# go-compression/raisin

Measured on AMD Instinct MI355X. Metric: encode+decode MB/s, higher is better.
Workload: dtype u8; 1 GPU; huffman encode+decode, 1024 MiB uniform-random bytes 0x00-0x7F (BASELINE configs[1]), splitmix64 seed 0x5EED0002; algorithm=huffman, bytes_per_gpu=1073741824, chunks=1

## Files before the change

### raisin_amd/csrc/huff_decode.hip

```cpp
#include <chrono>
#include <optional>
#include "codecs.h"
#include "rsn_helpers.h"

namespace rsn {


constexpr int DB = 256;
constexpr int FDB = 256;
constexpr int SW = 8;
constexpr int SBITS = SW * 32;
constexpr int ORG_WORDS = 8;
constexpr int ORG = ORG_WORDS * 32;
constexpr int DATA_WORDS = ORG_WORDS + DB * SW + 8;
constexpr int LUT_BITS_MAX = 11;
constexpr int LUT_WORDS = 1 << LUT_BITS_MAX;
constexpr int OUT_STAGE = DB * 64;
constexpr int OUT_STAGE_RUNE = 40960;
constexpr int CHILD_LDS = 256;
constexpr int LUT2_LDS = 768;
constexpr uint32_t LUT2_GLOBAL_MAX = 1u << 20;
constexpr int SYNC_ROUNDS = 24;
constexpr uint32_t BAD_REL = 0xFFFF;
constexpr uint32_t BAD_POS = 0xFFFFFFFFu;
// ... 582 lines not shown
        for (uint32_t k = 0; k < cnt; k++) dst[k] = (uint8_t)(o[k >> 2] >> (8 * (k & 3)));
    }
    }
    __syncthreads();
    }
}

namespace {

void build_tables(const HuffTree &t, int K, std::vector<uint32_t> &lut, std::vector<int32_t> &child) {
    const uint32_t A = t.n_leaves;
    const size_t n_int = t.freq.size() - A;
    child.assign(2 * std::max<size_t>(n_int, 1), 0);
    for (size_t i = 0; i < n_int; i++) {
        const int32_t id = (int32_t)(A + i);
        const int32_t kids[2] = {t.left[id], t.right[id]};
        for (int b = 0; b < 2; b++)
            child[2 * i + b] = t.is_leaf(kids[b]) ? -(int32_t)(t.rune[kids[b]] + 1) : kids[b] - (int32_t)A;
    }
    lut.assign((size_t)1 << K, 0);
    struct It { int32_t node; uint32_t prefix; int depth; };
    std::vector<It> st;
    st.push_back({t.root, 0, 0});
    while (!st.empty()) {
        const It it = st.back();
        st.pop_back();
        if (t.is_leaf(it.node)) {
            const uint32_t ent = ((uint32_t)it.depth << 24) | t.rune[it.node];
            const uint32_t lo = it.prefix << (K - it.depth);
            for (uint32_t x = 0; x < (1u << (K - it.depth)); x++) lut[lo + x] = ent;
        } else if (it.depth == K) {
            lut[it.prefix] = 0x80000000u | (uint32_t)(it.node - (int32_t)A);
        } else {
            st.push_back({t.right[it.node], (it.prefix << 1) | 1, it.depth + 1});
            st.push_back({t.left[it.node], it.prefix << 1, it.depth + 1});
        }
    }
}

void build_second_level(const std::vector<int32_t> &child, int K, bool byte_alphabet, std::vector<uint32_t> &lut, std::vector<uint32_t> &lut2) {
    lut2.clear();
    const size_t n_int = child.size() / 2;
    std::vector<uint8_t> depth(n_int, 0);
    for (size_t i = 0; i < n_int; i++) {
        unsigned d = 0;
        for (int b = 0; b < 2; b++) { const int32_t k = child[2 * i + b]; d = std::max(d, k < 0 ? 1u : 1u + depth[(size_t)k]); }
        depth[i] = (uint8_t)std::min(d, 255u);
    }
    std::vector<uint32_t> longs;
    for (uint32_t v = 0; v < (1u << K); v++) if (lut[v] & 0x80000000u) longs.push_back(v);
    if (longs.empty()) return;
    auto total = [&](unsigned cap) { uint64_t t = 0; for (uint32_t v : longs) t += 1ull << std::min<unsigned>(depth[lut[v] & 0x3FFFFFFu], cap); return t; };
    unsigned cap = 32u - (unsigned)K;
    if (total(cap) > (uint64_t)LUT2_LDS) {
        const uint64_t budget = byte_alphabet ? (uint64_t)LUT2_LDS : (uint64_t)LUT2_GLOBAL_MAX;
        while (cap > 0 && total(cap) > budget) cap--;
    }
    if (cap == 0) return;
    struct It { int32_t node; uint32_t path; unsigned q; };
    std::vector<It> st;
    for (uint32_t v : longs) {
        const int32_t top = (int32_t)(lut[v] & 0x3FFFFFFu);
        const unsigned sb = std::min<unsigned>(depth[(size_t)top], cap);
        const uint32_t off = (uint32_t)lut2.size();
        lut2.resize(lut2.size() + ((size_t)1 << sb));
        st.push_back({top, 0, 0});
        while (!st.empty()) {
            const It it = st.back();
            st.pop_back();
            if (it.q == sb) { lut2[off + it.path] = 0x80000000u | (uint32_t)it.node; continue; }
            for (int b = 0; b < 2; b++) {
                const int32_t k = child[2 * (size_t)it.node + b];
                const uint32_t path = it.path | ((uint32_t)b << it.q);
                const unsigned q1 = it.q + 1;
                if (k >= 0) { st.push_back({k, path, q1}); continue; }
                const uint32_t ent = ((uint32_t)(K + q1) << 24) | (uint32_t)(-(k + 1));
                for (uint32_t y = 0; y < (1u << (sb - q1)); y++) lut2[off + path + (y << q1)] = ent;
            }
        }
        lut[v] = 0x80000000u | (sb << 26) | off;
    }
}

int rep_for(int K) {
    int r = 0;
    while (r < 5 && ((1 << K) << (r + 1)) <= LUT_WORDS) r++;
    return r;
}

}

int huff_decode_dev(Ctx &c, hipStream_t s, const uint8_t *d_in, size_t n, uint8_t *d_out, size_t out_cap, size_t *out_n, const SliceStream *st) {
    if (((uintptr_t)d_in & 15) || ((uintptr_t)d_out & 15)) return c.fail(RSN_ERR_ARG, "huffman: device buffers must be 16-byte aligned");
    *out_n = 0;
    std::vector<uint8_t> head;
    size_t sep = (size_t)-1;
    for (size_t want = 4096;; want *= 8) {
        const size_t k = std::min(want, n);
        const size_t old = head.size();
        if (k > old) {
            if (st && !st->need_in(k)) return c.fail(RSN_ERR_DEVICE, "huffman: the upload of a sliced call failed");
            void *hpin; int prc = pinned_buf(c, k - old + 64, &hpin); if (prc) return prc;
            RSN_HIP(copy_async(hpin, d_in + old, k - old, hipMemcpyDeviceToHost, s));
            RSN_HIP(hipStreamSynchronize(s));
            head.resize(k);
            memcpy(head.data() + old, hpin, k - old);
        }
        for (size_t i = old ? old - 1 : 0; i + 1 < k; i++) if (head[i] == 0x5C && head[i + 1] == 0x0A) { sep = i; break; }
        if (sep != (size_t)-1 || k == n) break;
    }
    if (sep == (size_t)-1) return c.fail(RSN_ERR_FORMAT, "huffman: no '\\\\\\n' separator (reference: index out of range, huffman.go:264)");
    if (sep + 3 > head.size() && sep + 3 <= n) {
        const size_t old = head.size();
        if (st && !st->need_in(sep + 3)) return c.fail(RSN_ERR_DEVICE, "huffman: the upload of a sliced call failed");
        void *hpin; int prc = pinned_buf(c, 64, &hpin); if (prc) return prc;
        RSN_HIP(copy_async(hpin, d_in + old, sep + 3 - old, hipMemcpyDeviceToHost, s));
        RSN_HIP(hipStreamSynchronize(s));
        head.resize(sep + 3);
        memcpy(head.data() + old, hpin, sep + 3 - old);
    }
    std::vector<HuffSym> syms; std::string msg;
    static const bool host_timing = getenv("RSN_HOST_TIMING") != nullptr;
    auto now = [] { return std::chrono::steady_clock::now(); };
    auto ms = [](std::chrono::steady_clock::time_point a, std::chrono::steady_clock::time_point b) { return std::chrono::duration<double, std::milli>(b - a).count(); };
    const auto t0 = now();
    if (!parse_header(head.data(), sep, syms, msg)) return c.fail(RSN_ERR_FORMAT, "%s", msg.c_str());
    const auto t1 = now();
    const size_t sn = n - sep - 2;
    const unsigned diff = sn ? head[sep + 2] : 0;
    const unsigned long long nbits = sn ? (unsigned long long)(sn - 1) * 8 : 0;
    if (diff > nbits) return c.fail(RSN_ERR_FORMAT, "huffman: pad exceeds the payload (reference: slice bounds out of range, huffman.go:294)");
    const unsigned long long max = nbits - diff;
    if (!d_out) {
        if (syms.empty()) return c.fail(RSN_ERR_FORMAT, "huffman: empty header (reference panics in heap.Pop, huffman.go:102)");
        if (syms.size() == 1) {
            if (max > 0) return c.fail(RSN_ERR_FORMAT, "huffman: single-symbol tree with a non-empty payload (reference recurses without end, huffman.go:139-140)");
            *out_n = 32;
            return c.fail(RSN_ERR_CAPACITY, "huffman: output needs %d bytes by the header's counts", utf8_len(syms[0].rune));
        }
        if (max == 0) return c.fail(RSN_ERR_FORMAT, "huffman: payload ends inside a codeword (reference: index out of range, huffman.go:145)");
        unsigned long long total = 0, expect = 0;
        bool beyond = false;
        for (const HuffSym &sy : syms) {
            if (sy.freq > max - total) { beyond = true; break; }
            total += sy.freq;
            expect += sy.freq * (unsigned long long)utf8_len(sy.rune);
        }
        if (beyond) expect = 4 * max;
        *out_n = round_up((size_t)expect, 16) + 16;
        return c.fail(RSN_ERR_CAPACITY, beyond ? "huffman: output needs at most %llu bytes (the header counts more symbols than the payload holds)"
                                               : "huffman: output needs %llu bytes by the header's counts", expect);
    }
    HuffTree tree; HuffCodes codes;
    if (!build_tree(syms, tree, msg)) return c.fail(RSN_ERR_FORMAT, "%s", msg.c_str());
    const auto t2 = now();
    constexpr int k_env = LUT_BITS_MAX;
    std::vector<uint32_t> lut, lut2; std::vector<int32_t> child;
    const bool prebuilt = tree.n_leaves > 4096;
    std::optional<SideJob> table_builder;
    if (prebuilt) table_builder.emplace([&] { build_tables(tree, k_env, lut, child); build_second_level(child, k_env, false, lut, lut2); });
    const bool codes_ok = assign_codes(tree, codes, msg, false);
    if (prebuilt) table_builder->finish();
    if (!codes_ok) return c.fail(RSN_ERR_LIMIT, "%s", msg.c_str());
    const auto t3 = now();
    if (host_timing) fprintf(stderr, "huffman decode host: header of %zu bytes parsed in %.2f ms, tree %.2f ms, codes %.2f ms, %zu symbols\n", sep, ms(t0, t1), ms(t1, t2), ms(t2, t3), syms.size());

    if (tree.n_leaves == 1) {
        if (max > 0) return c.fail(RSN_ERR_FORMAT, "huffman: single-symbol tree with a non-empty payload (reference recurses without end, huffman.go:139-140)");
        uint8_t u[4];
        const size_t k = (size_t)go_encode_rune(tree.rune[0], u);
        *out_n = k;
        if (!d_out || out_cap < k) { return c.fail(RSN_ERR_CAPACITY, "huffman: output needs %zu bytes", k); }
        RSN_HIP(copy_async(d_out, u, k, hipMemcpyHostToDevice, s));
        RSN_HIP(hipStreamSynchronize(s));
        return RSN_OK;
    }
    if (max == 0) return c.fail(RSN_ERR_FORMAT, "huffman: payload ends inside a codeword (reference: index out of range, huffman.go:145)");

    bool ascii = true;
    for (uint32_t i = 0; i < tree.n_leaves; i++) if (tree.rune[i] >= 0x80) ascii = false;
    const size_t pay = sep + 3;
    const size_t A0 = pay & ~(size_t)15;
    void *p; int rc;

    static const bool no_flat = getenv("RSN_NO_FLAT") != nullptr;
    if (ascii && codes.min_len == codes.max_len && codes.max_len <= 7 && !no_flat) {
        const uint32_t L = codes.max_len;
        if (max % L) return c.fail(RSN_ERR_FORMAT, "huffman: payload ends inside a codeword (reference: index out of range, huffman.go:145)");
        const unsigned long long n_sym = max / L;
// ... 284 lines not shown
```

### raisin_amd/csrc/huff_encode.hip

```cpp
#include <chrono>
#include <cstddef>

#include <optional>
#include "codecs.h"
#include "rsn_helpers.h"

namespace rsn {

constexpr int TILE = 65536;
constexpr int SMALL_TILE = 4096;
constexpr size_t SMALL_INPUT = (size_t)2 << 20;
constexpr size_t RUNE_SMALL_INPUT = (size_t)16 << 20;
constexpr int HB = 256;
constexpr int ROUND = HB * 16;

enum { MODE_ASCII = 0, MODE_ASCII_WIDE = 1, MODE_RUNE = 2 };

template <int INFLIGHT, int TB>
__global__ __launch_bounds__(HB) void k_byte_hist(const uint8_t *__restrict__ in, size_t n, uint32_t n_tiles,
                                                  uint32_t *__restrict__ tile_hist,
                                                  unsigned long long *__restrict__ ghist) {
    __shared__ uint32_t h[128 * 32];
    const int tid = threadIdx.x;
    const uint32_t copy = tid & 31;
    unsigned long long mine = 0;
    uint32_t hi_any = 0;
    static_assert(TB % ROUND == 0 && (TB / ROUND) % INFLIGHT == 0, "whole rounds, whole batches of loads");
    auto add16 = [&](const uint4 &v) {
        const uint32_t w[4] = {v.x, v.y, v.z, v.w};
#pragma unroll
        for (int j = 0; j < 4; j++) {
            hi_any |= w[j];
            atomicAdd(&h[((w[j] & 0x7F) << 5) | copy], 1u);
            atomicAdd(&h[(((w[j] >> 8) & 0x7F) << 5) | copy], 1u);
            atomicAdd(&h[(((w[j] >> 16) & 0x7F) << 5) | copy], 1u);
            atomicAdd(&h[(((w[j] >> 24) & 0x7F) << 5) | copy], 1u);
        }
    };
    for (uint32_t t = blockIdx.x; t < n_tiles; t += gridDim.x) {
        for (int i = tid; i < 128 * 32; i += HB) h[i] = 0;
        __syncthreads();
        const size_t base = (size_t)t * TB;
        if (base + TB <= n) {
            const uint4 *src = reinterpret_cast<const uint4 *>(in + base) + tid;
#pragma unroll
            for (int k0 = 0; k0 < TB / ROUND; k0 += INFLIGHT) {
                uint4 v[INFLIGHT];
#pragma unroll
                for (int k = 0; k < INFLIGHT; k++) v[k] = ld16<(RSN_NT_MASK & 1) != 0>(src + (k0 + k) * HB);
#pragma unroll
                for (int k = 0; k < INFLIGHT; k++) add16(v[k]);
            }
        } else {
            for (int k = 0; k < TB / ROUND; k++) {
                const size_t off = base + (size_t)(k * HB + tid) * 16;
                if (off + 16 <= n) add16(*reinterpret_cast<const uint4 *>(in + off));
                else if (off < n) for (size_t p = off; p < n; p++) { hi_any |= in[p]; atomicAdd(&h[((in[p] & 0x7F) << 5) | copy], 1u); }
            }
        }
        __syncthreads();
        if (tid < 128) {
            uint32_t s = 0;
#pragma unroll
            for (int r = 0; r < 32; r++) s += h[(tid << 5) | ((r + tid) & 31)];
            tile_hist[(size_t)t * 128 + tid] = s;
            mine += s;
        }
        __syncthreads();
    }
    if (tid < 128 && mine) atomicAdd(&ghist[tid], mine);
    if (hi_any & 0x80808080u) atomicAdd(&ghist[128], 1ull);
}

template <int COPIES, int INFLIGHT>
__global__ __launch_bounds__(HB) void k_byte_hist256(const uint8_t *__restrict__ in, size_t n, uint32_t n_tiles,
                                                     unsigned long long *__restrict__ ghist) {
    static_assert(HB == 256 && (COPIES == 16 || COPIES == 32) && (TILE / ROUND) % INFLIGHT == 0, "a thread per bin, whole batches of loads");
    constexpr uint32_t FOLD = 1024;
    constexpr int LOG = COPIES == 32 ? 5 : 4;
    __shared__ uint32_t h[256 * COPIES];
    const int tid = threadIdx.x;
    const uint32_t copy = tid & (COPIES - 1);
    unsigned long long mine = 0;
    auto add16 = [&](const uint4 &v) {
        const uint32_t w[4] = {v.x, v.y, v.z, v.w};
#pragma unroll
        for (int j = 0; j < 4; j++) {
            atomicAdd(&h[((w[j] & 0xFF) << LOG) | copy], 1u);
            atomicAdd(&h[(((w[j] >> 8) & 0xFF) << LOG) | copy], 1u);
            atomicAdd(&h[(((w[j] >> 16) & 0xFF) << LOG) | copy], 1u);
            atomicAdd(&h[((w[j] >> 24) << LOG) | copy], 1u);
        }
    };
    auto fold = [&] {
        __syncthreads();
        uint32_t s = 0;
#pragma unroll
        for (int r = 0; r < COPIES; r++) s += h[(tid << LOG) | ((r + tid) & (COPIES - 1))];
        mine += s;
        __syncthreads();
        for (int i = tid; i < 256 * COPIES; i += HB) h[i] = 0;
        __syncthreads();
    };
    for (int i = tid; i < 256 * COPIES; i += HB) h[i] = 0;
    __syncthreads();
    uint32_t since = 0;
    for (uint32_t t = blockIdx.x; t < n_tiles; t += gridDim.x) {
        const size_t base = (size_t)t * TILE;
        if (base + TILE <= n) {
            const uint4 *src = reinterpret_cast<const uint4 *>(in + base) + tid;
#pragma unroll
            for (int k0 = 0; k0 < TILE / ROUND; k0 += INFLIGHT) {
                uint4 v[INFLIGHT];
#pragma unroll
                for (int k = 0; k < INFLIGHT; k++) v[k] = ld16<true>(src + (k0 + k) * HB);
#pragma unroll
                for (int k = 0; k < INFLIGHT; k++) add16(v[k]);
            }
        } else {
            for (int k = 0; k < TILE / ROUND; k++) {
                const size_t off = base + (size_t)(k * HB + tid) * 16;
                if (off + 16 <= n) add16(*reinterpret_cast<const uint4 *>(in + off));
                else if (off < n) for (size_t p = off; p < n; p++) atomicAdd(&h[((uint32_t)in[p] << LOG) | copy], 1u);
            }
        }
        if (++since == FOLD) { fold(); since = 0; }
    }
    fold();
    if (mine) atomicAdd(&ghist[tid], mine);
}

template <int INFLIGHT>
__global__ __launch_bounds__(HB) void k_bytes_differ(const uint8_t *__restrict__ a, const uint8_t *__restrict__ b, size_t n, uint32_t n_tiles,
                                                     unsigned long long *__restrict__ first) {
    static_assert((TILE / ROUND) % INFLIGHT == 0, "whole batches of loads");
    constexpr unsigned long long NONE = ~0ull;
    __shared__ unsigned long long s_pub, s_min;
    const int tid = threadIdx.x;
    auto diff16 = [](const uint4 &x, const uint4 &y) -> uint32_t {
        const uint32_t d[4] = {x.x ^ y.x, x.y ^ y.y, x.z ^ y.z, x.w ^ y.w};
        uint32_t at = 16;
#pragma unroll
        for (int j = 3; j >= 0; j--) if (d[j]) at = 4 * j + ((uint32_t)__ffs((int)d[j]) - 1) / 8;
        return at;
    };
    for (uint32_t t = blockIdx.x; t < n_tiles; t += gridDim.x) {
        const size_t base = (size_t)t * TILE;
        if (tid == 0) { s_pub = __hip_atomic_load(first, __ATOMIC_RELAXED, __HIP_MEMORY_SCOPE_AGENT); s_min = NONE; }
        __syncthreads();
        if (base >= s_pub) return;
        unsigned long long mine = NONE;
        if (base + TILE <= n) {
            const uint4 *pa = reinterpret_cast<const uint4 *>(a + base) + tid, *pb = reinterpret_cast<const uint4 *>(b + base) + tid;
#pragma unroll
// ... 624 lines not shown
            const int bp = k * L, wi = bp >> 5, sh = bp & 31;
            if (sh + L <= 32) v[wi] |= code << (32 - sh - L);
            else { v[wi] |= code >> (sh + L - 32); v[wi + 1 < L ? wi + 1 : wi] |= code << (64 - sh - L); }
        }
    };
    uint32_t v[L];
    if (s0 < a.n) pack32(s0, v);
    else {
#pragma unroll
        for (int j = 0; j < L; j++) v[j] = 0;
    }
    uint32_t prev = (uint32_t)__builtin_amdgcn_update_dpp(0, (int)v[L - 1], 0x138, 0xF, 0xF, false);
    if (lane == 63) s_last[wv] = v[L - 1];
    __syncthreads();
    if (lane == 0) {
        if (wv > 0) prev = s_last[wv - 1];
        else if (chunk > 0) { uint32_t pv[L]; pack32(s0 - 32, pv); prev = pv[L - 1]; }
        else prev = 0;
    }
    const uint32_t o0 = (uint32_t)(a.base_bits & 31);
#pragma unroll
    for (int j = 0; j < L; j++) {
        const uint32_t hi = j ? v[j - 1] : prev;
        const uint32_t ow = (uint32_t)((((unsigned long long)hi << 32) | v[j]) >> o0);
        const uint32_t i = tid * L + j;
        s_o[i + (i >> 5)] = __builtin_bswap32(ow);
    }
    __syncthreads();
    const unsigned long long total_syms = a.n;
    const unsigned long long wbase = (a.base_bits >> 5) + (unsigned long long)chunk * (HB * L);
    const unsigned long long end_word = (a.base_bits + total_syms * L + 31) >> 5;
    if (chunk > 0 && wbase + (unsigned long long)(HB * L) <= end_word) {
        for (int q = tid; q < HB * L / 4; q += HB) {
            const int i = 4 * q;
            const uint32_t *sp = s_o + i + (i >> 5);
            st16_a4<(RSN_NT_MASK & 4) != 0>(a.out_words + wbase + i, sp[0], sp[1], sp[2], sp[3]);
        }
    } else
    for (int i = tid; i < HB * L; i += HB) {
        const unsigned long long g = wbase + i;
        if (g >= end_word) break;
        const uint32_t val = s_o[i + (i >> 5)];
        if (g == (a.base_bits >> 5)) {
            uint32_t hb = 0;
            for (uint32_t k = (uint32_t)(g * 4); k < a.hdr_len; k++) hb |= (uint32_t)tab[128 + k] << (8 * (k & 3));
            a.out_words[g] = val | hb;
        } else a.out_words[g] = val;
    }
    if (o0 && tid == HB - 1) {
        const unsigned long long g = wbase + (unsigned long long)(HB * L);
        const bool last_block = chunk + 1 == n_chunks;
        if (last_block && g < end_word) a.out_words[g] = __builtin_bswap32(v[L - 1] << (32 - o0));
    }
    __syncthreads();
    }
    if (blockIdx.x == 0) {
        const uint32_t whole = (uint32_t)(a.base_bits >> 5) * 4;
        uint8_t *o8 = reinterpret_cast<uint8_t *>(a.out_words);
        for (uint32_t k = tid; k < whole && k < a.hdr_len; k += HB) o8[k] = tab[128 + k];
    }
}

namespace {

__global__ void k_rune_flags(const unsigned long long *__restrict__ hist, unsigned long long *__restrict__ flag) {
    const uint32_t r = blockIdx.x * blockDim.x + threadIdx.x;
    if (r < kMaxRune) flag[r] = hist[r] != 0;
}
__global__ void k_rune_pairs(const unsigned long long *__restrict__ hist, const unsigned long long *__restrict__ off, HuffSym *__restrict__ out) {
    const uint32_t r = blockIdx.x * blockDim.x + threadIdx.x;
    if (r < kMaxRune && hist[r]) { out[off[r]].rune = r; out[off[r]].freq = hist[r]; }
}
struct RuneCode { uint32_t rune, len; unsigned long long code; };
__global__ void k_rune_table(const RuneCode *__restrict__ list, uint32_t k, unsigned long long *__restrict__ code64, uint8_t *__restrict__ len8) {
    const uint32_t i = blockIdx.x * blockDim.x + threadIdx.x;
    if (i < k) { const RuneCode e = list[i]; code64[e.rune] = e.code; len8[e.rune] = (uint8_t)e.len; }
}

int hist_ascii_or_rune(Ctx &c, hipStream_t s, const uint8_t *d_in, size_t n, uint32_t n_tiles, uint32_t tile, uint32_t *d_tile_hist,
                       std::vector<HuffSym> &syms, bool &ascii, uint16_t **smask_out) {
    void *p;
    int rc = dev_buf(c, 1, 256 * 8, &p); if (rc) return rc;
    unsigned long long *d_gh = (unsigned long long *)p;
    RSN_HIP(hipMemsetAsync(d_gh, 0, 256 * 8, s));
    dim3 grid;
    if (tile == TILE) {
        rc = persistent_grid(c, reinterpret_cast<const void *>(k_byte_hist<4, TILE>), HB, n_tiles, &grid); if (rc) return rc;
        RSN_LAUNCH("huff_byte_hist", (k_byte_hist<4, TILE>), grid, dim3(HB), 0, s, d_in, n, n_tiles, d_tile_hist, d_gh);
    } else {
        rc = persistent_grid(c, reinterpret_cast<const void *>(k_byte_hist<1, SMALL_TILE>), HB, n_tiles, &grid); if (rc) return rc;
        RSN_LAUNCH("huff_byte_hist", (k_byte_hist<1, SMALL_TILE>), grid, dim3(HB), 0, s, d_in, n, n_tiles, d_tile_hist, d_gh);
    }
    void *hp; rc = pinned_buf(c, 256 * 8, &hp); if (rc) return rc;
    unsigned long long *h = (unsigned long long *)hp;
    RSN_HIP(copy_async(h, d_gh, 256 * 8, hipMemcpyDeviceToHost, s));
    RSN_HIP(hipStreamSynchronize(s));
    ascii = h[128] == 0;
    syms.clear();
    if (ascii) {
        for (uint32_t b = 0; b < 128; b++) if (h[b]) syms.push_back({b, h[b]});
        return RSN_OK;
    }
    rc = dev_buf(c, 2, (size_t)kMaxRune * 8, &p); if (rc) return rc;
    unsigned long long *d_rh = (unsigned long long *)p;
    RSN_HIP(hipMemsetAsync(d_rh, 0, (size_t)kMaxRune * 8, s));
    const size_t rounds = ceil_div(n, ROUND);
    uint16_t *d_smask = nullptr;
    { rc = dev_buf(c, 26, (ceil_div(n, 16) + 2) * 2 + 64, &p); if (rc) return rc; d_smask = (uint16_t *)p; }
    *smask_out = d_smask;
    RSN_LAUNCH("huff_rune_hist", k_rune_hist, dim3((uint32_t)std::min<size_t>(rounds, 4096)), dim3(HB), 0, s, d_in, n, d_rh, d_smask);
    const size_t bound = std::min<size_t>(n, kMaxRune);
    rc = dev_buf(c, 6, (size_t)kMaxRune * 16 + 16 + bound * sizeof(HuffSym) + 64, &p); if (rc) return rc;
    unsigned long long *d_flag = (unsigned long long *)p, *d_off = d_flag + kMaxRune, *d_cnt = d_off + kMaxRune;
    HuffSym *d_pairs = (HuffSym *)(d_cnt + 2);
    const dim3 rg((kMaxRune + 255) / 256);
    RSN_LAUNCH("huff_rune_hist", k_rune_flags, rg, dim3(256), 0, s, d_rh, d_flag);
    rc = scan_u64(c, s, "huff_scan", d_flag, d_off, kMaxRune, d_cnt); if (rc) return rc;
    RSN_LAUNCH("huff_rune_hist", k_rune_pairs, rg, dim3(256), 0, s, d_rh, d_off, d_pairs);
    const bool one_trip = bound * sizeof(HuffSym) <= (1u << 20);
    rc = pinned_buf(c, 16 + (one_trip ? bound * sizeof(HuffSym) : 0), &hp); if (rc) return rc;
    h = (unsigned long long *)hp;
    RSN_HIP(copy_async(h, d_cnt, 16 + (one_trip ? bound * sizeof(HuffSym) : 0), hipMemcpyDeviceToHost, s));
    RSN_HIP(hipStreamSynchronize(s));
    const size_t present = (size_t)h[0];
    if (!one_trip) {
        rc = pinned_buf(c, 16 + present * sizeof(HuffSym), &hp); if (rc) return rc;
        h = (unsigned long long *)hp;
        RSN_HIP(copy_async(h + 2, d_pairs, present * sizeof(HuffSym), hipMemcpyDeviceToHost, s));
        RSN_HIP(hipStreamSynchronize(s));
    }
    const HuffSym *hs = reinterpret_cast<const HuffSym *>(h + 2);
    syms.assign(hs, hs + present);
    return RSN_OK;
}

}

size_t huff_compress_bound(size_t n) {
    const size_t syms = std::min<size_t>(n, kMaxRune);
    return n * 21 / 8 + syms * 26 + 96;
}

int huff_slice_hist(Ctx &c, hipStream_t s, const uint8_t *d_in, size_t n, HuffSlice &sl) {
    sl.tile = n <= SMALL_INPUT ? SMALL_TILE : TILE;
    sl.n_tiles = (uint32_t)ceil_div(n, sl.tile);
    void *p;
    int rc = dev_buf(c, 0, (size_t)sl.n_tiles * 128 * 4, &p); if (rc) return rc;
    sl.d_tile_hist = (uint32_t *)p;
    sl.d_smask = nullptr;
    rc = hist_ascii_or_rune(c, s, d_in, n, sl.n_tiles, sl.tile, sl.d_tile_hist, sl.syms, sl.ascii, &sl.d_smask); if (rc) return rc;
    if (!sl.ascii && n <= RUNE_SMALL_INPUT) {
        sl.tile = SMALL_TILE;
        sl.n_tiles = (uint32_t)ceil_div(n, sl.tile);
    }
    return RSN_OK;
}

int huff_slice_emit(Ctx &c, hipStream_t s, const uint8_t *d_in, size_t n, const HuffSlice &sl, const HuffTree &tree, const HuffCodes &codes, bool flat,
                    const std::string &hdr, unsigned long long base_bits, unsigned long long slice_bits, uint8_t *d_out) {
    void *p; int rc;
    const size_t H = hdr.size();
    const uint32_t tile = sl.tile, n_tiles = sl.n_tiles;
    if (slice_bits == 0) {
        if (H) RSN_HIP(copy_async(d_out, hdr.data(), H, hipMemcpyHostToDevice, s));
        RSN_HIP(hipStreamSynchronize(s));
        return RSN_OK;
    }

    if (flat) {
        const unsigned L = codes.max_len;
        FlatEmitArgs fa{};
        fa.in = d_in; fa.n = n; fa.base_bits = base_bits; fa.out_words = (uint32_t *)d_out; fa.hdr_len = (uint32_t)H;
        uint8_t *hcodes = fa.inl;
        if (128 + H > (size_t)FE_INLINE) {
            void *hp2; rc = pinned_buf(c, 128 + H + 16, &hp2); if (rc) return rc;
            hcodes = (uint8_t *)hp2;
            memset(hcodes, 0, 128);
        }
        for (uint32_t i = 0; i < tree.n_leaves; i++) hcodes[tree.rune[i]] = (uint8_t)codes.code[i];
// ... 127 lines not shown
```

### raisin_amd/csrc/rsn_api.hip

```cpp
#include "codecs.h"
#include "rsn_common.h"
#include "rsn_helpers.h"

#include <sys/mman.h>

#include <algorithm>
#include <atomic>
#include <cmath>
#include <chrono>
#include <condition_variable>
#include <functional>
#include <mutex>
#include <thread>

namespace rsn {

namespace {
int env_int(const char *name, int dflt) { const char *e = getenv(name); return e && *e ? atoi(e) : dflt; }
std::atomic<size_t> g_arena_bytes[64];
}

Ctx &ctx() {
    static thread_local Ctx c;
    return c;
}

namespace {
struct Parked {
    int device; hipStream_t stream; Ctx::Buf bufs[Ctx::N_BUFS]; void *pinned; size_t pinned_cap; std::vector<hipEvent_t> events;
};
std::mutex g_park_mu;
std::vector<Parked> *g_parked = nullptr;

void release_parked(Parked &pk) {
    if (hipSetDevice(pk.device) != hipSuccess) return;
    for (auto &b : pk.bufs) if (b.p) { (void)hipFree(b.p); g_arena_bytes[pk.device & 63] -= b.cap; }
    if (pk.pinned) (void)hipHostFree(pk.pinned);
    for (auto e : pk.events) (void)hipEventDestroy(e);
    if (pk.stream) (void)hipStreamDestroy(pk.stream);
}

size_t max_parked() {
    static const size_t v = [] {
        if (getenv("RSN_MAX_PARKED")) return (size_t)std::max(0, atoi(getenv("RSN_MAX_PARKED")));
        int cnt = 0;
        if (hipGetDeviceCount(&cnt) != hipSuccess || cnt < 0) cnt = 0;
        return (size_t)(8 + 3 * cnt);
    }();
    return v;
}

void trim_parked_excess(int restore_device) {
    std::vector<Parked> victims;
    {
        std::lock_guard<std::mutex> lk(g_park_mu);
        if (!g_parked) return;
        while (g_parked->size() > max_parked()) { victims.push_back(std::move(g_parked->front())); g_parked->erase(g_parked->begin()); }
    }
    if (victims.empty()) return;
    for (auto &pk : victims) release_parked(pk);
    (void)hipSetDevice(restore_device);
}

std::atomic<unsigned> g_rr{0};
int default_device(int cnt) {
    const char *e = getenv("RSN_DEVICE");
    if (!e || !*e) return 0;
    if (!strcmp(e, "rr") || !strcmp(e, "all")) return (int)(g_rr.fetch_add(1) % (unsigned)cnt);
    return atoi(e);
}
}

Ctx::~Ctx() {
    if (!inited) return;
    std::lock_guard<std::mutex> lk(g_park_mu);
    if (!g_parked) g_parked = new std::vector<Parked>();
    Parked pk;
    pk.device = device; pk.stream = own_stream; pk.pinned = pinned; pk.pinned_cap = pinned_cap;
    for (int i = 0; i < N_BUFS; i++) pk.bufs[i] = bufs[i];
    pk.events = free_events;
    for (auto &sl : slots) for (auto &pr : sl.pending) { pk.events.push_back(pr.first); pk.events.push_back(pr.second); }
    g_parked->push_back(std::move(pk));
}

int ctx_init(Ctx &c) {
    if (c.inited) {
        hipError_t e = hipSetDevice(c.device);
        if (e != hipSuccess) return c.fail(RSN_ERR_DEVICE, "hipSetDevice(%d): %s", c.device, hipGetErrorString(e));
        return RSN_OK;
    }
    int cnt = 0;
    hipError_t e = hipGetDeviceCount(&cnt);
    if (e != hipSuccess || cnt <= 0)
        return c.fail(RSN_ERR_DEVICE, "no HIP device available (%s); librsn has no CPU fallback", e != hipSuccess ? hipGetErrorString(e) : "device count 0");
    if (!c.device_chosen) { c.device = default_device(cnt); c.device_chosen = true; }
    if (c.device < 0 || c.device >= cnt) return c.fail(RSN_ERR_DEVICE, "device %d out of range (%d visible)", c.device, cnt);
    RSN_HIP(hipSetDevice(c.device));
    trim_parked_excess(c.device);
    {
        std::lock_guard<std::mutex> lk(g_park_mu);
        if (g_parked)
            for (size_t i = g_parked->size(); i-- > 0;)
                if ((*g_parked)[i].device == c.device) {
                    Parked &pk = (*g_parked)[i];
                    if (c.pinned) (void)hipHostFree(c.pinned);
                    c.own_stream = pk.stream; c.pinned = pk.pinned; c.pinned_cap = pk.pinned_cap;
                    for (int k = 0; k < Ctx::N_BUFS; k++) c.bufs[k] = pk.bufs[k];
                    c.free_events = std::move(pk.events);
                    g_parked->erase(g_parked->begin() + (long)i);
                    c.inited = true;
                    return RSN_OK;
                }
    }
    RSN_HIP(hipStreamCreateWithFlags(&c.own_stream, hipStreamNonBlocking));
    c.inited = true;
    return RSN_OK;
}

namespace {
struct ScratchGate { std::mutex mu; std::condition_variable cv; size_t cap = 0, in_flight = 0; int calls = 0, waiting = 0; unsigned long long queued = 0; };
ScratchGate g_gate[64];
}

size_t scratch_admit(Ctx &c, size_t need) {
    if (c.gate_held || need == 0) return 0;
    ScratchGate &g = g_gate[c.device & 63];
    std::unique_lock<std::mutex> lk(g.mu);
    if (g.cap == 0) {
        const char *e = getenv("RSN_SCRATCH_GIB");
        size_t fr = 0, tot = 0;
        if (e && atof(e) > 0) g.cap = (size_t)(atof(e) * (double)((size_t)1 << 30));
        else if (hipMemGetInfo(&fr, &tot) == hipSuccess && tot) g.cap = tot / 100 * 85;
        else g.cap = (size_t)64 << 30;
    }
    if (g.calls > 0 && g.in_flight + need > g.cap) {
        static const bool dbg = getenv("RSN_SCRATCH_DEBUG") != nullptr;
        g.waiting++; g.queued++;
        if (dbg) fprintf(stderr, "librsn: a call that needs %.2f GiB of scratch waits: %d in flight need %.2f of %.2f GiB\n", need / 1073741824.0, g.calls, g.in_flight / 1073741824.0, g.cap / 1073741824.0);
        g.cv.wait(lk, [&] { return g.calls == 0 || g.in_flight + need <= g.cap; });
        g.waiting--;
    }
    g.calls++; g.in_flight += need;
    c.gate_held = need;
    return need;
}

void scratch_release(Ctx &c, size_t need, unsigned long long slots) {
    if (need == 0) return;
    c.gate_held = 0;
    ScratchGate &g = g_gate[c.device & 63];
    bool give_back;
    {
        std::lock_guard<std::mutex> lk(g.mu);
        g.calls--; g.in_flight -= need;
        give_back = g.waiting > 0 || g_arena_bytes[c.device & 63].load() > g.cap / 2;
    }
    if (give_back && hipSetDevice(c.device) == hipSuccess) {
        for (int k = 0; k < Ctx::N_BUFS; k++) {
            if (!((slots >> k) & 1ull)) continue;
            Ctx::Buf &b = c.bufs[k];
            if (b.p && b.cap >= ((size_t)64 << 20)) { (void)hipFree(b.p); g_arena_bytes[c.device & 63] -= b.cap; b.p = nullptr; b.cap = 0; }
        }
    }
    g.cv.notify_all();
}

void scratch_forget(Ctx &c, size_t bytes) { g_arena_bytes[c.device & 63] -= bytes; }
unsigned long long scratch_queued(int device) { ScratchGate &g = g_gate[device & 63]; std::lock_guard<std::mutex> lk(g.mu); return g.queued; }

static void trim_own_context() {
    Ctx &c = ctx();
    if (c.inited && hipSetDevice(c.device) == hipSuccess) {
        (void)hipStreamSynchronize(c.own_stream);
        for (auto &b : c.bufs) { if (b.p) { (void)hipFree(b.p); g_arena_bytes[c.device & 63] -= b.cap; } b.p = nullptr; b.cap = 0; }
        if (c.pinned) (void)hipHostFree(c.pinned);
        c.pinned = nullptr; c.pinned_cap = 0;
    }
}

int dev_buf(Ctx &c, int slot, size_t bytes, void **out) {
    Ctx::Buf &b = c.bufs[slot];
    if (bytes > b.cap) {
        if (b.p) { RSN_HIP(hipFree(b.p)); g_arena_bytes[c.device & 63] -= b.cap; b.p = nullptr; b.cap = 0; }
        const size_t want = round_up(bytes + bytes / 8, 4096);
        hipError_t e = hipMalloc(&b.p, want);
        if (e != hipSuccess) {
            (void)hipGetLastError();
            std::vector<Parked> victims;
            { std::lock_guard<std::mutex> lk(g_park_mu); if (g_parked) victims.swap(*g_parked); }
            for (auto &pk : victims) release_parked(pk);
            HelperPool::on_idle(trim_own_context);
            (void)hipSetDevice(c.device);
            e = hipMalloc(&b.p, want);
        }
        if (e != hipSuccess) { b.p = nullptr; return c.fail(RSN_ERR_NOMEM, "hipMalloc(%zu): %s", want, hipGetErrorString(e)); }
        b.cap = want;
        static std::atomic<unsigned long long> next_gen{0};
        b.gen = ++next_gen;
        g_arena_bytes[c.device & 63] += want;
    }
    *out = b.p;
    return RSN_OK;
}

int pinned_buf(Ctx &c, size_t bytes, void **out) {
    if (bytes > c.pinned_cap) {
        if (c.pinned) { RSN_HIP(hipHostFree(c.pinned)); c.pinned = nullptr; c.pinned_cap = 0; }
        hipError_t e = hipHostMalloc(&c.pinned, bytes, hipHostMallocDefault);
        if (e != hipSuccess) { c.pinned = nullptr; return c.fail(RSN_ERR_NOMEM, "hipHostMalloc(%zu): %s", bytes, hipGetErrorString(e)); }
        c.pinned_cap = bytes;
    }
    *out = c.pinned;
    return RSN_OK;
}

int func_dyn_lds(Ctx &c, const void *fn, size_t bytes) {
    static std::mutex mu;
    static std::vector<std::pair<std::pair<const void *, int>, size_t>> *seen = new std::vector<std::pair<std::pair<const void *, int>, size_t>>();
    std::lock_guard<std::mutex> lk(mu);
    for (auto &e : *seen)
        if (e.first.first == fn && e.first.second == c.device) {
            if (bytes <= e.second) return RSN_OK;
            RSN_HIP(hipFuncSetAttribute(fn, hipFuncAttributeMaxDynamicSharedMemorySize, (int)bytes));
            e.second = bytes;
            return RSN_OK;
        }
    RSN_HIP(hipFuncSetAttribute(fn, hipFuncAttributeMaxDynamicSharedMemorySize, (int)bytes));
    seen->push_back({{fn, c.device}, bytes});
    return RSN_OK;
}

void prof_collect(Ctx &c) {
    for (auto &sl : c.slots) {
        for (auto &pr : sl.pending) {
            float ms = 0;
            if (hipEventSynchronize(pr.second) == hipSuccess && hipEventElapsedTime(&ms, pr.first, pr.second) == hipSuccess) {
                sl.total_ms += ms;
                sl.launches++;
            }
            c.free_events.push_back(pr.first);
            c.free_events.push_back(pr.second);
        }
        sl.pending.clear();
    }
}

namespace {

constexpr size_t RES_HDR = 64, POOL_MIN = 1u << 20;
constexpr size_t POOL_BLOCKS = 12;
struct ResHdr { unsigned long long magic, cap; };
constexpr unsigned long long RES_MAGIC = 0x52534E5F52455330ull;
std::mutex g_pool_mu;
std::vector<std::pair<size_t, void *>> g_pool;

bool pool_enabled() { return true; }

void *result_alloc(size_t n) {
    const size_t need = n ? n : 1;
// ... 1374 lines not shown
```

### raisin_amd/csrc/rsn_common.h

```cpp
#pragma once

#include <hip/hip_runtime.h>

#include <cstdarg>
#include <cstdint>
#include <cstdio>
#include <cstdlib>
#include <cstring>
#include <algorithm>
#include <atomic>
#include <mutex>
#include <string>
#include <vector>

#include "../../include/rsn.h"

namespace rsn {

struct ProfSlot {
    std::string name;
    uint64_t launches = 0;
    double total_ms = 0;
    std::vector<std::pair<hipEvent_t, hipEvent_t>> pending;
};

struct Ctx {
    int device = 0;
    bool device_chosen = false;
    bool inited = false;
    hipStream_t own_stream = nullptr;
    std::string err;
    bool prof = false;
    std::vector<ProfSlot> slots;
    std::vector<hipEvent_t> free_events;

    struct Buf { void *p = nullptr; size_t cap = 0; unsigned long long gen = 0; };
    enum { N_BUFS = 43 };
    Buf bufs[N_BUFS];
    void *pinned = nullptr; size_t pinned_cap = 0;
    bool lz_runs = false;
    size_t gate_held = 0;

    ~Ctx();

    int fail(int code, const char *fmt, ...) {
        char tmp[512];
        va_list ap; va_start(ap, fmt); vsnprintf(tmp, sizeof tmp, fmt, ap); va_end(ap);
        err = tmp;
        return code;
    }
};

Ctx &ctx();
int ctx_init(Ctx &c);
int dev_buf(Ctx &c, int slot, size_t bytes, void **out);
int pinned_buf(Ctx &c, size_t bytes, void **out);
size_t scratch_admit(Ctx &c, size_t need);
void scratch_release(Ctx &c, size_t held, unsigned long long slots);
void scratch_forget(Ctx &c, size_t bytes);
unsigned long long scratch_queued(int device);
void prof_collect(Ctx &c);
int func_dyn_lds(Ctx &c, const void *fn, size_t bytes);

#define RSN_HIP(call)                                                                              \
    do {                                                                                           \
        hipError_t e__ = (call);                                                                   \
        if (e__ != hipSuccess)                                                                     \
            return c.fail(RSN_ERR_DEVICE, "%s failed: %s (%s:%d)", #call, hipGetErrorString(e__),  \
                          __FILE__, __LINE__);                                                     \
    } while (0)

inline int persistent_grid(Ctx &c, const void *fn, int block, size_t work, dim3 *grid) {
    struct Entry { const void *fn; int device, block; uint32_t blocks; };
    static std::mutex mu;
    static std::vector<Entry> *seen = new std::vector<Entry>();
    uint32_t blocks = 0;
    {
        std::lock_guard<std::mutex> lk(mu);
        for (const Entry &e : *seen)
            if (e.fn == fn && e.device == c.device && e.block == block) { blocks = e.blocks; break; }
        if (!blocks) {
            int per_cu = 0, cus = 0;
            RSN_HIP(hipOccupancyMaxActiveBlocksPerMultiprocessor(&per_cu, fn, block, 0));
            RSN_HIP(hipDeviceGetAttribute(&cus, hipDeviceAttributeMultiprocessorCount, c.device));
            if (per_cu < 1 || cus < 1) return c.fail(RSN_ERR_DEVICE, "occupancy query: %d blocks of %d threads a CU on %d CUs", per_cu, block, cus);
            blocks = (uint32_t)per_cu * (uint32_t)cus;
            seen->push_back({fn, c.device, block, blocks});
        }
    }
    *grid = dim3((uint32_t)std::min<size_t>(work, blocks));
    return RSN_OK;
}

struct CopyCount { std::atomic<int> on{0}; std::atomic<unsigned long long> h2d{0}, d2h{0}; };
inline CopyCount g_copy_count;
inline hipError_t copy_async(void *dst, const void *src, size_t bytes, hipMemcpyKind kind, hipStream_t s) {
    if (g_copy_count.on.load(std::memory_order_relaxed)) {
        if (kind == hipMemcpyHostToDevice) g_copy_count.h2d.fetch_add(bytes, std::memory_order_relaxed);
        else if (kind == hipMemcpyDeviceToHost) g_copy_count.d2h.fetch_add(bytes, std::memory_order_relaxed);
    }
    return hipMemcpyAsync(dst, src, bytes, kind, s);
}

struct ProfScope {
    Ctx &c; hipStream_t s; int slot = -1; hipEvent_t a = nullptr, b = nullptr;
    ProfScope(Ctx &c_, hipStream_t s_, const char *name) : c(c_), s(s_) {
        if (!c.prof) return;
        for (size_t i = 0; i < c.slots.size(); i++) if (c.slots[i].name == name) slot = (int)i;
        if (slot < 0) { c.slots.emplace_back(); c.slots.back().name = name; slot = (int)c.slots.size() - 1; }
        auto get = [&]() { hipEvent_t e = nullptr; if (!c.free_events.empty()) { e = c.free_events.back(); c.free_events.pop_back(); } else (void)hipEventCreate(&e); return e; };
        a = get(); b = get();
        (void)hipEventRecord(a, s);
    }
    ~ProfScope() {
        if (slot < 0) return;
        (void)hipEventRecord(b, s);
        c.slots[slot].pending.emplace_back(a, b);
    }
};

#define RSN_LAUNCH(name, kernel, grid, block, shmem, stream, ...)                                  \
    do {                                                                                           \
        {                                                                                          \
            rsn::ProfScope ps__(c, stream, name);                                                  \
            hipLaunchKernelGGL(kernel, grid, block, shmem, stream, __VA_ARGS__);                   \
        }                                                                                          \
        RSN_HIP(hipGetLastError());                                                                \
    } while (0)

#ifndef RSN_NT_MASK
#define RSN_NT_MASK 1
#endif
#ifdef __HIPCC__
typedef uint32_t rsn_u32x4 __attribute__((ext_vector_type(4)));
typedef uint32_t rsn_u32x4_a4 __attribute__((ext_vector_type(4), aligned(4)));
template <bool NT> __device__ __forceinline__ uint4 ld16(const uint4 *p) {
    if constexpr (NT) { const rsn_u32x4 v = __builtin_nontemporal_load(reinterpret_cast<const rsn_u32x4 *>(p)); return make_uint4(v.x, v.y, v.z, v.w); }
    else return *p;
}
template <bool NT> __device__ __forceinline__ uint32_t ld4(const uint32_t *p) {
    if constexpr (NT) return __builtin_nontemporal_load(p);
    else return *p;
}
template <bool NT> __device__ __forceinline__ void st16(uint4 *p, const uint4 &v) {
    if constexpr (NT) { rsn_u32x4 x = {v.x, v.y, v.z, v.w}; __builtin_nontemporal_store(x, reinterpret_cast<rsn_u32x4 *>(p)); }
    else *p = v;
}
template <bool NT> __device__ __forceinline__ void st16_a4(uint32_t *p, uint32_t a, uint32_t b, uint32_t c_, uint32_t d) {
    rsn_u32x4_a4 x = {a, b, c_, d};
    if constexpr (NT) __builtin_nontemporal_store(x, reinterpret_cast<rsn_u32x4_a4 *>(p));
    else *reinterpret_cast<rsn_u32x4_a4 *>(p) = x;
}
#endif

static inline size_t ceil_div(size_t a, size_t b) { return (a + b - 1) / b; }
static inline size_t round_up(size_t a, size_t b) { return ceil_div(a, b) * b; }

}
```

Before: 1.001 million MB/s.

## Post small device results to pinned host memory instead of memcpy+sync

Adds a pinned-host post area that kernels write directly with system-scope stores plus a sequence flag, which the host spin-waits on. The encode histogram's last block (found by a ticket counter) writes the global histogram and resets it, so the next call can skip the memset. The decode header probe is copied by a tiny kernel into the post area. Both replace a D2H memcpy plus stream synchronize. The intent is to cut per-call host round-trip latency, at the cost of host spinning and extra cross-call state that tracks whether the histogram buffer is already clean.

```diff
diff --git a/raisin_amd/csrc/huff_decode.hip b/raisin_amd/csrc/huff_decode.hip
--- a/raisin_amd/csrc/huff_decode.hip
+++ b/raisin_amd/csrc/huff_decode.hip
@@ -688,6 +688,14 @@
     }
 }
 
+__global__ __launch_bounds__(256) void k_post_head(const uint8_t *__restrict__ in, uint32_t k, uint8_t *__restrict__ post,
+                                                   unsigned long long *__restrict__ seq_word, unsigned long long seq) {
+    const uint32_t at = threadIdx.x * 16;
+    if (at + 16 <= k) *reinterpret_cast<uint4 *>(post + at) = *reinterpret_cast<const uint4 *>(in + at);
+    else for (uint32_t i = at; i < k; i++) post[i] = in[i];
+    post_raise(seq_word, seq);
+}
+
 int rep_for(int K) {
     int r = 0;
     while (r < 5 && ((1 << K) << (r + 1)) <= LUT_WORDS) r++;
@@ -706,11 +714,20 @@
         const size_t old = head.size();
         if (k > old) {
             if (st && !st->need_in(k)) return c.fail(RSN_ERR_DEVICE, "huffman: the upload of a sliced call failed");
-            void *hpin; int prc = pinned_buf(c, k - old + 64, &hpin); if (prc) return prc;
-            RSN_HIP(copy_async(hpin, d_in + old, k - old, hipMemcpyDeviceToHost, s));
-            RSN_HIP(hipStreamSynchronize(s));
-            head.resize(k);
-            memcpy(head.data() + old, hpin, k - old);
+            if (old == 0 && k <= POST_BYTES && post_enabled()) {
+                PostArea *pa; int prc = post_area(c, &pa); if (prc) return prc;
+                const unsigned long long seq = post_next_seq();
+                hipLaunchKernelGGL(k_post_head, dim3(1), dim3(256), 0, s, d_in, (uint32_t)k, pa->payload, &pa->seq, seq);
+                RSN_HIP(hipGetLastError());
+                prc = post_wait(c, s, pa, seq); if (prc) return prc;
+                head.assign(pa->payload, pa->payload + k);
+            } else {
+                void *hpin; int prc = pinned_buf(c, k - old + 64, &hpin); if (prc) return prc;
+                RSN_HIP(copy_async(hpin, d_in + old, k - old, hipMemcpyDeviceToHost, s));
+                RSN_HIP(hipStreamSynchronize(s));
+                head.resize(k);
+                memcpy(head.data() + old, hpin, k - old);
+            }
         }
         for (size_t i = old ? old - 1 : 0; i + 1 < k; i++) if (head[i] == 0x5C && head[i + 1] == 0x0A) { sep = i; break; }
         if (sep != (size_t)-1 || k == n) break;
diff --git a/raisin_amd/csrc/huff_encode.hip b/raisin_amd/csrc/huff_encode.hip
--- a/raisin_amd/csrc/huff_encode.hip
+++ b/raisin_amd/csrc/huff_encode.hip
@@ -16,10 +16,12 @@
 
 enum { MODE_ASCII = 0, MODE_ASCII_WIDE = 1, MODE_RUNE = 2 };
 
+constexpr int GH_TICKET = 255;
 template <int INFLIGHT, int TB>
 __global__ __launch_bounds__(HB) void k_byte_hist(const uint8_t *__restrict__ in, size_t n, uint32_t n_tiles,
                                                   uint32_t *__restrict__ tile_hist,
-                                                  unsigned long long *__restrict__ ghist) {
+                                                  unsigned long long *__restrict__ ghist,
+                                                  unsigned long long *__restrict__ post, unsigned long long seq) {
     __shared__ uint32_t h[128 * 32];
     const int tid = threadIdx.x;
     const uint32_t copy = tid & 31;
@@ -70,6 +72,11 @@
     }
     if (tid < 128 && mine) atomicAdd(&ghist[tid], mine);
     if (hi_any & 0x80808080u) atomicAdd(&ghist[128], 1ull);
+    if (post && post_last_block(reinterpret_cast<uint32_t *>(ghist + GH_TICKET))) {
+        if (tid <= 128) post[tid] = atomicExch(&ghist[tid], 0ull);
+        if (tid == 0) atomicExch(reinterpret_cast<uint32_t *>(ghist + GH_TICKET), 0u);
+        post_raise(post + POST_BYTES / 8, seq);
+    }
 }
 
 template <int COPIES, int INFLIGHT>
@@ -860,19 +867,32 @@
     void *p;
     int rc = dev_buf(c, 1, 256 * 8, &p); if (rc) return rc;
     unsigned long long *d_gh = (unsigned long long *)p;
-    RSN_HIP(hipMemsetAsync(d_gh, 0, 256 * 8, s));
+    const bool post = post_enabled();
+    PostArea *pa = nullptr;
+    unsigned long long seq = 0, *d_post = nullptr;
+    if (post) { rc = post_area(c, &pa); if (rc) return rc; seq = post_next_seq(); d_post = reinterpret_cast<unsigned long long *>(pa->payload); }
+    if (!post || c.hist_clean_gen != c.bufs[1].gen) RSN_HIP(hipMemsetAsync(d_gh, 0, 256 * 8, s));
+    c.hist_clean_gen = 0;
     dim3 grid;
     if (tile == TILE) {
         rc = persistent_grid(c, reinterpret_cast<const void *>(k_byte_hist<4, TILE>), HB, n_tiles, &grid); if (rc) return rc;
-        RSN_LAUNCH("huff_byte_hist", (k_byte_hist<4, TILE>), grid, dim3(HB), 0, s, d_in, n, n_tiles, d_tile_hist, d_gh);
+        RSN_LAUNCH("huff_byte_hist", (k_byte_hist<4, TILE>), grid, dim3(HB), 0, s, d_in, n, n_tiles, d_tile_hist, d_gh, d_post, seq);
     } else {
         rc = persistent_grid(c, reinterpret_cast<const void *>(k_byte_hist<1, SMALL_TILE>), HB, n_tiles, &grid); if (rc) return rc;
-        RSN_LAUNCH("huff_byte_hist", (k_byte_hist<1, SMALL_TILE>), grid, dim3(HB), 0, s, d_in, n, n_tiles, d_tile_hist, d_gh);
-    }
-    void *hp; rc = pinned_buf(c, 256 * 8, &hp); if (rc) return rc;
-    unsigned long long *h = (unsigned long long *)hp;
-    RSN_HIP(copy_async(h, d_gh, 256 * 8, hipMemcpyDeviceToHost, s));
-    RSN_HIP(hipStreamSynchronize(s));
+        RSN_LAUNCH("huff_byte_hist", (k_byte_hist<1, SMALL_TILE>), grid, dim3(HB), 0, s, d_in, n, n_tiles, d_tile_hist, d_gh, d_post, seq);
+    }
+    void *hp;
+    unsigned long long *h;
+    if (post) {
+        rc = post_wait(c, s, pa, seq); if (rc) return rc;
+        c.hist_clean_gen = c.bufs[1].gen;
+        h = d_post;
+    } else {
+        rc = pinned_buf(c, 256 * 8, &hp); if (rc) return rc;
+        h = (unsigned long long *)hp;
+        RSN_HIP(copy_async(h, d_gh, 256 * 8, hipMemcpyDeviceToHost, s));
+        RSN_HIP(hipStreamSynchronize(s));
+    }
     ascii = h[128] == 0;
     syms.clear();
     if (ascii) {
diff --git a/raisin_amd/csrc/rsn_api.hip b/raisin_amd/csrc/rsn_api.hip
--- a/raisin_amd/csrc/rsn_api.hip
+++ b/raisin_amd/csrc/rsn_api.hip
@@ -27,7 +27,7 @@
 
 namespace {
 struct Parked {
-    int device; hipStream_t stream; Ctx::Buf bufs[Ctx::N_BUFS]; void *pinned; size_t pinned_cap; std::vector<hipEvent_t> events;
+    int device; hipStream_t stream; Ctx::Buf bufs[Ctx::N_BUFS]; void *pinned; size_t pinned_cap; void *post; std::vector<hipEvent_t> events;
 };
 std::mutex g_park_mu;
 std::vector<Parked> *g_parked = nullptr;
@@ -36,6 +36,7 @@
     if (hipSetDevice(pk.device) != hipSuccess) return;
     for (auto &b : pk.bufs) if (b.p) { (void)hipFree(b.p); g_arena_bytes[pk.device & 63] -= b.cap; }
     if (pk.pinned) (void)hipHostFree(pk.pinned);
+    if (pk.post) (void)hipHostFree(pk.post);
     for (auto e : pk.events) (void)hipEventDestroy(e);
     if (pk.stream) (void)hipStreamDestroy(pk.stream);
 }
@@ -76,7 +77,7 @@
     std::lock_guard<std::mutex> lk(g_park_mu);
     if (!g_parked) g_parked = new std::vector<Parked>();
     Parked pk;
-    pk.device = device; pk.stream = own_stream; pk.pinned = pinned; pk.pinned_cap = pinned_cap;
+    pk.device = device; pk.stream = own_stream; pk.pinned = pinned; pk.pinned_cap = pinned_cap; pk.post = post;
     for (int i = 0; i < N_BUFS; i++) pk.bufs[i] = bufs[i];
     pk.events = free_events;
     for (auto &sl : slots) for (auto &pr : sl.pending) { pk.events.push_back(pr.first); pk.events.push_back(pr.second); }
@@ -104,7 +105,9 @@
                 if ((*g_parked)[i].device == c.device) {
                     Parked &pk = (*g_parked)[i];
                     if (c.pinned) (void)hipHostFree(c.pinned);
-                    c.own_stream = pk.stream; c.pinned = pk.pinned; c.pinned_cap = pk.pinned_cap;
+                    if (c.post) (void)hipHostFree(c.post);
+                    c.own_stream = pk.stream; c.pinned = pk.pinned; c.pinned_cap = pk.pinned_cap; c.post = pk.post;
+                    c.hist_clean_gen = 0;
                     for (int k = 0; k < Ctx::N_BUFS; k++) c.bufs[k] = pk.bufs[k];
                     c.free_events = std::move(pk.events);
                     g_parked->erase(g_parked->begin() + (long)i);
@@ -175,6 +178,8 @@
         for (auto &b : c.bufs) { if (b.p) { (void)hipFree(b.p); g_arena_bytes[c.device & 63] -= b.cap; } b.p = nullptr; b.cap = 0; }
         if (c.pinned) (void)hipHostFree(c.pinned);
         c.pinned = nullptr; c.pinned_cap = 0;
+        if (c.post) (void)hipHostFree(c.post);
+        c.post = nullptr;
     }
 }
 
diff --git a/raisin_amd/csrc/rsn_common.h b/raisin_amd/csrc/rsn_common.h
--- a/raisin_amd/csrc/rsn_common.h
+++ b/raisin_amd/csrc/rsn_common.h
@@ -9,6 +9,7 @@
 #include <cstring>
 #include <algorithm>
 #include <atomic>
+#include <chrono>
 #include <mutex>
 #include <string>
 #include <vector>
@@ -38,6 +39,8 @@
     enum { N_BUFS = 43 };
     Buf bufs[N_BUFS];
     void *pinned = nullptr; size_t pinned_cap = 0;
+    void *post = nullptr;
+    unsigned long long hist_clean_gen = 0;
     bool lz_runs = false;
     size_t gate_held = 0;
 
@@ -102,6 +105,36 @@
     return hipMemcpyAsync(dst, src, bytes, kind, s);
 }
 
+constexpr size_t POST_BYTES = 4096;
+constexpr int POST_SPIN_MS = 5;
+struct PostArea { uint8_t payload[POST_BYTES]; unsigned long long seq; };
+inline bool post_enabled() { static const bool on = getenv("RSN_NO_POST") == nullptr; return on; }
+inline unsigned long long post_next_seq() { static std::atomic<unsigned long long> next{0}; return ++next; }
+inline int post_area(Ctx &c, PostArea **out) {
+    if (!c.post) {
+        hipError_t e = hipHostMalloc(&c.post, sizeof(PostArea) + 56, hipHostMallocDefault);
+        if (e != hipSuccess) { c.post = nullptr; return c.fail(RSN_ERR_NOMEM, "hipHostMalloc(%zu): %s", sizeof(PostArea) + 56, hipGetErrorString(e)); }
+        memset(c.post, 0, sizeof(PostArea) + 56);
+    }
+    *out = (PostArea *)c.post;
+    return RSN_OK;
+}
+inline int post_wait(Ctx &c, hipStream_t s, const PostArea *pa, unsigned long long seq) {
+    const volatile unsigned long long *w = &pa->seq;
+    const auto t0 = std::chrono::steady_clock::now();
+    for (uint32_t spins = 1;; spins++) {
+        if (*w == seq) { std::atomic_thread_fence(std::memory_order_acquire); return RSN_OK; }
+        if ((spins & 1023) == 0 && std::chrono::steady_clock::now() - t0 > std::chrono::milliseconds(POST_SPIN_MS)) {
+            RSN_HIP(hipStreamSynchronize(s));
+            if (*w != seq) return c.fail(RSN_ERR_DEVICE, "a kernel finished without posting its result to the host");
+            std::atomic_thread_fence(std::memory_order_acquire);
+            return RSN_OK;
+        }
+#if defined(__x86_64__) || defined(__i386__)
+        __builtin_ia32_pause();
+#endif
+    }
+}
 struct ProfScope {
     Ctx &c; hipStream_t s; int slot = -1; hipEvent_t a = nullptr, b = nullptr;
     ProfScope(Ctx &c_, hipStream_t s_, const char *name) : c(c_), s(s_) {
@@ -146,6 +179,19 @@
     if constexpr (NT) { rsn_u32x4 x = {v.x, v.y, v.z, v.w}; __builtin_nontemporal_store(x, reinterpret_cast<rsn_u32x4 *>(p)); }
     else *p = v;
 }
+__device__ __forceinline__ bool post_last_block(uint32_t *ticket) {
+    __shared__ uint32_t s_post_last;
+    __threadfence();
+    __syncthreads();
+    if (threadIdx.x == 0) s_post_last = atomicAdd(ticket, 1u) == gridDim.x - 1;
+    __syncthreads();
+    return s_post_last != 0;
+}
+__device__ __forceinline__ void post_raise(unsigned long long *seq_word, unsigned long long seq) {
+    __threadfence_system();
+    __syncthreads();
+    if (threadIdx.x == 0) __hip_atomic_store(seq_word, seq, __ATOMIC_RELEASE, __HIP_MEMORY_SCOPE_SYSTEM);
+}
 template <bool NT> __device__ __forceinline__ void st16_a4(uint32_t *p, uint32_t a, uint32_t b, uint32_t c_, uint32_t d) {
     rsn_u32x4_a4 x = {a, b, c_, d};
     if constexpr (NT) __builtin_nontemporal_store(x, reinterpret_cast<rsn_u32x4_a4 *>(p));
```

Measured after the change: 856,400 MB/s. -14.4%, worse.
